# do-mpc/do-mpc

Hardware: AMD Instinct MI355X
Metric: MPC steps/sec (make_step wall-time), industrial_poly robust multi-stage (higher is better)
Workload: dtype f64

## Files before the change

__graft_entry__.py:

```python
import os
import subprocess
import sys

ROOT = os.path.dirname(os.path.abspath(__file__))
if ROOT not in sys.path:
    sys.path.insert(0, ROOT)

PREBUILT = [
    ("oscillating_masses", {}),
    ("batch_reactor", {}),
    ("batch_reactor", {"n_horizon": 50}),
    ("CSTR", {}),
    ("CSTR", {"n_robust": 0, "collocation_deg": 3}),
    ("CSTR", {"track_sign": -3000.0}),
    ("industrial_poly", {}),
    ("industrial_poly", {"n_robust": 2, "uncertainty": "paired"}),
    ("industrial_poly", {"collocation_deg": 3, "collocation_ni": 2, "n_horizon": 6}),
    ("kinematic_bicycle", {}),
    ("dynamic_bicycle", {}),
    ("kite", {"n_horizon": 20}),
    ("rotating_masses", {}),
    ("CSTR", {"custom_rterm": "default_as_expression"}),
    ("CSTR", {"custom_rterm": "custom"}),
    ("oscillating_masses", {"custom_rterm": "custom"}),
    ("oscillating_masses_dae", {}),
    ("dip", {}),
    ("CSTR", {"n_robust": 0, "nl_cons_check_colloc_points": True}),
    ("dip", {"n_horizon": 40, "nl_cons_check_colloc_points": True}),
    ("CSTR", {"nl_cons_single_slack": True}),
    ("CSTR", {"nl_cons_single_slack": True, "n_robust": 2, "n_horizon": 8, "uncertainty": {"alpha": [1.0, 1.05, 0.95], "beta": [1.0]}}),
    ("CSTR", {"nl_cons_single_slack": True, "n_robust": 0, "nl_cons_check_colloc_points": True}),
    ("CSTR", {"open_loop": True, "uncertainty": {"alpha": [1.0, 1.05, 0.95], "beta": [1.0]}}),
    ("CSTR", {"open_loop": True, "n_robust": 2, "n_horizon": 6, "uncertainty": {"alpha": [1.0, 1.05], "beta": [1.0]}, "soft_T_R": False}),
    ("shape_family:s1", {}), ("shape_family:s2", {}), ("shape_family:s3", {}), ("shape_family:s4", {}), ("shape_family:s5", {}),
    ("shape_family:s6", {}), ("shape_family:s7", {}), ("shape_family:s8", {}), ("shape_family:s9", {}),
]

PREBUILT_BATCH = [
    ("industrial_poly", {}), ("industrial_poly", {"n_robust": 2, "uncertainty": "paired"}),
    ("oscillating_masses", {}), ("CSTR", {}), ("CSTR", {"n_robust": 0, "collocation_deg": 3}), ("batch_reactor", {}), ("batch_reactor", {"n_horizon": 50}),
    ("rotating_masses", {}),
]
PREBUILT_BATCH_MHE = [("rotating_masses", "build_mhe", {}, {}), ("rotating_masses", "build_mhe_w", {"process_noise": True}, {}),
                      ("rotating_masses", "build_mhe_w", {"process_noise": True}, {"scaling": "MHE_W_SCALING"})]


PREBUILT_DEFS = [("CSTR", {}, "DOMPC_FORCE_DENSE=1"), ("batch_reactor", {}, "DOMPC_FORCE_DENSE=1"),
                 ("CSTR", {}, "DOMPC_GJ_U=1e9"), ("industrial_poly", {}, "DOMPC_GJ_U=1e9"),
                 ("batch_reactor", {}, "DOMPC_REG_GJ=0"), ("batch_reactor", {}, "DOMPC_GJ_U=1e9"),
                 ("industrial_poly", {}, "DOMPC_QUAD=0"), ("CSTR", {}, "DOMPC_QUAD=0"), ("CSTR", {"n_horizon": 5, "n_robust": 0}, "DOMPC_QUAD=0")]

PREBUILT_NODE_PACK = [("industrial_poly", {}), ("CSTR", {})] + [("shape_family:s%d" % i, {}) for i in range(1, 10)]
PREBUILT_BATCH_FAMILY = [("shape_family:s%d" % i, {}) for i in range(1, 10)]

PREBUILT_QUAD_LDS = [("DOMPC_QUAD_LDS=1", [("industrial_poly", {}), ("CSTR", {})]),
                     ("DOMPC_GJ_U=1e9", [("industrial_poly", {})]),
                     ("DOMPC_GJ_U=1e9 DOMPC_QUAD_LDS=1", [("industrial_poly", {})])]


PREBUILT_SHARD = [
    ("CSTR", {}),
    ("industrial_poly", {"n_robust": 2, "uncertainty": "paired"}),
]


PREBUILT_MHE = [("rotating_masses", "build_mhe", {}, {}), ("rotating_masses", "build_mhe_w", {"process_noise": True}, {}),
                ("rotating_masses", "build_mhe_w", {"process_noise": True}, {"scaling": "MHE_W_SCALING"}),
                ("rotating_masses", "build_mhe", {"dae": True}, {}), ("rotating_masses", "build_mhe_w", {"process_noise": True, "dae": True}, {}),
                ("oscillating_masses", "build_mhe", {"estimation": True}, {}), ("oscillating_masses", "build_mhe", {"estimation": True, "dae": True}, {}),
                ("rotating_masses", "build_mhe_w", {"process_noise": True}, {"soft_limit": (-0.1, 0.01)}),
                ("rotating_masses", "build_mhe_w", {"process_noise": True}, {"soft_limit": (-0.1, 0.01), "nl_cons_single_slack": True}),
                ("rotating_masses", "build_mhe_w", {"process_noise": True, "input_meas_noise": False}, {})]


PREBUILT_ROUTE = [("oscillating_masses", "docstring", False, False), ("oscillating_masses", "tree", False, False),
                  ("industrial_poly", "tree", False, True), ("CSTR", "tree", False, True), ("batch_reactor", "tree", False, False),
                  ("oscillating_masses_dae", "tree", False, False), ("rotating_masses", "tree", False, False),
                  ("CSTR", "docstring", False, False), ("batch_reactor", "docstring", False, False), ("industrial_poly", "docstring", False, False),
                  ("oscillating_masses", None, True, False), ("CSTR", None, True, False), ("CSTR", "tree", True, False),
                  ("industrial_poly", None, True, False), ("industrial_poly", "tree", True, False), ("batch_reactor", None, True, False),
                  ("rotating_masses", None, True, False)]


def lowered_route_cases():
    from do_mpc_amd import controller
    from do_mpc_amd.examples import CASES
    tests = os.path.join(ROOT, "tests")
    if tests not in sys.path:
        sys.path.insert(0, tests)
    import route_cases as rc
    out = []
    orig = controller.HipIpmSolver
    controller.HipIpmSolver = _NoSolver
    try:
        for name, cost, rows, batch in PREBUILT_ROUTE:
            ex = CASES[name]
            mpc = rc.stopped_before_setup(lambda n: ex.build_mpc(ex.build_model()), name)
            mpc.prepare_nlp()
            if rows:
                rc.rows_at_three_nodes(mpc, name)
            if cost:
                rc.ADDED_COST[cost](mpc)
            mpc.create_nlp()
            out.append((f"{name} + {cost or ''}{' + rows' if rows else ''} (low-level route)", {}, mpc.generated_header, mpc.model_hash, batch))
    finally:
        controller.HipIpmSolver = orig
    return out


PREBUILT_PLANTS = ["oscillating_masses", "batch_reactor", "CSTR", "industrial_poly", "oscillating_masses_dae", "dip", "rotating_masses",
                   "triple_tank", "batch_reactor_lqr_dae", "batch_reactor_lqr_dae:build_dae_model"]

PREBUILT_EKF = [("triple_tank", {}), ("oscillating_masses", {"estimation": True}), ("rotating_masses", {}), ("CSTR", {})]


def lowered_ekf(entries=None):
    from do_mpc_amd.ekf import EKF
    from do_mpc_amd.examples import CASES
    out = []
    for name, kw in (PREBUILT_EKF if entries is None else entries):
        hdr = EKF(CASES[name].build_model(**kw))._lower()
        out.append((name, kw, hdr, hdr.rsplit('EKF_MODEL_HASH "', 1)[1].split('"')[0]))
    return out


PREBUILT_EKF_DAE = ["masses", "nonlinear_discrete", "continuous", "dip", "batch_reactor", "limit", "status", "oscillating_masses_dae",
                    "masses_eliminated", "batch_reactor_eliminated"]


def lowered_ekf_dae(entries=None):
    tests = os.path.join(ROOT, "tests")
    if tests not in sys.path:
        sys.path.insert(0, tests)
    import ekf_dae_common as dc
    out = []
    for name in (PREBUILT_EKF_DAE if entries is None else entries):
        hdr = dc.make_filter(name)._lower()
        out.append((name, hdr, hdr.rsplit('EKF_MODEL_HASH "', 1)[1].split('"')[0]))
    return out


# ... 68 lines not shown

def lowered_asmpc(entries=None):
    from do_mpc_amd import lowering
    out = []
    for nx, nu in (PREBUILT_ASMPC if entries is None else entries):
        hdr = lowering.lower_asmpc(nx, nu)
        out.append((f"n_x = {nx}, n_u = {nu}", hdr, hdr.rsplit('ASMPC_MODEL_HASH "', 1)[1].split('"')[0]))
    return out


class _NoSolver:

    def __init__(self, *a, **k):
        pass


def lowered_models(which=None):
    from do_mpc_amd import controller
    from do_mpc_amd.examples import CASES
    out = []
    orig = controller.HipIpmSolver
    controller.HipIpmSolver = _NoSolver
    try:
        for name, kw in (PREBUILT if which is None else which):
            ex = CASES[name]
            mpc = ex.build_mpc(ex.build_model(), **kw)
            out.append((name, kw, mpc.generated_header, mpc.model_hash))
        if which is None:
            out += _lower_mhe(PREBUILT_MHE)
    finally:
        controller.HipIpmSolver = orig
    return out


def _lower_mhe(entries):
    from do_mpc_amd.examples import CASES
    out = []
    for name, builder, mkw, bkw in entries:
        ex = CASES[name]
        bkw = {k: (getattr(ex, v) if isinstance(v, str) else v) for k, v in bkw.items()}
        mhe = getattr(ex, builder)(ex.build_model(**mkw), **bkw)
        out.append((f"{name} ({builder})", {**mkw, **{k: "..." for k in bkw}}, mhe._mpc.generated_header, mhe._mpc.model_hash))
    return out


def lowered_mhe(entries):
    from do_mpc_amd import controller
    orig = controller.HipIpmSolver
    controller.HipIpmSolver = _NoSolver
    try:
        return _lower_mhe(entries)
    finally:
        controller.HipIpmSolver = orig


def build() -> None:
    from do_mpc_amd import build as nb
    import do_mpc_amd
    from concurrent.futures import ThreadPoolExecutor
    lib = nb.runtime_library()
    print("[build] runtime:", lib)
    jobs = [(name, kw, header, h, False, False) for name, kw, header, h in lowered_models()]
    jobs += [(name, kw, header, h, True, False) for name, kw, header, h in lowered_models(PREBUILT_SHARD)]
    jobs += [(name, kw, header, h, False, True) for name, kw, header, h in lowered_models(PREBUILT_BATCH + PREBUILT_BATCH_FAMILY)]
    jobs += [(name, kw, header, h, False, True) for name, kw, header, h in lowered_mhe(PREBUILT_BATCH_MHE)]
    route = lowered_route_cases()
    jobs += [(name, kw, header, h, False, False) for name, kw, header, h, _ in route]
    jobs += [(name, kw, header, h, False, True) for name, kw, header, h, batch in route if batch]
    with ThreadPoolExecutor(max_workers=max(1, min(len(jobs), (os.cpu_count() or 2) - 1))) as pool:
        outs = list(pool.map(lambda j: nb.model_code_object(j[2], j[3], shard=j[4], batch_only=j[5]), jobs))
    for (name, kw, _, _, shard, batch), co in zip(jobs, outs):
        print(f"[build] {name} {kw}{' (tree sharding)' if shard else ''}{' (batch only)' if batch else ''}: {co}")
    for name, kw, defs in PREBUILT_DEFS:
        saved = os.environ.get("DOMPC_DEFS")
        os.environ["DOMPC_DEFS"] = defs
        try:
            for _, _, header, h in lowered_models([(name, kw)]):
                print(f"[build] {name} {kw} [{defs}]: {nb.model_code_object(header, h)}")
        finally:
            if saved is None:
                del os.environ["DOMPC_DEFS"]
            else:
                os.environ["DOMPC_DEFS"] = saved
    for defs, classes in [("DOMPC_NODE_PACK=0", PREBUILT_NODE_PACK)] + PREBUILT_QUAD_LDS:
        saved = os.environ.get("DOMPC_DEFS")
        os.environ["DOMPC_DEFS"] = defs
        try:
            jobs = [(name, kw, header, h, batch) for name, kw, header, h in lowered_models(classes) for batch in (False, True)]
            with ThreadPoolExecutor(max_workers=max(1, min(len(jobs), (os.cpu_count() or 2) - 1))) as pool:
                outs = list(pool.map(lambda j: nb.model_code_object(j[2], j[3], batch_only=j[4]), jobs))
            for (name, kw, _, _, batch), co in zip(jobs, outs):
                print(f"[build] {name} {kw} [{defs}]{' (batch only)' if batch else ''}: {co}")
        finally:
            if saved is None:
                del os.environ["DOMPC_DEFS"]
            else:
                os.environ["DOMPC_DEFS"] = saved
    from do_mpc_amd.examples import CASES
    from do_mpc_amd.simulator import Simulator
    for name in PREBUILT_PLANTS:
        case, _, builder = name.partition(":")
        hdr = Simulator(getattr(CASES[case], builder or "build_model")())._lower()
        co = nb.plant_code_object(hdr, hdr.rsplit('PLANT_MODEL_HASH "', 1)[1].split('"')[0])
        print(f"[build] plant {name}: {co}")
    failed = []
    for entry in PREBUILT_EKF:
        try:
            for name, kw, hdr, h in lowered_ekf([entry]):
                print(f"[build] filter {name} {kw}: {nb.ekf_code_object(hdr, h)}")
        except Exception as e:
            failed.append(entry)
            print(f"[build] filter {entry[0]} {entry[1]}: FAILED\n{e}")
    for entry in PREBUILT_EKF_DAE:
        try:
            for name, hdr, h in lowered_ekf_dae([entry]):
                print(f"[build] filter of a model with algebraic states '{name}': {nb.ekf_code_object(hdr, h)}")
        except Exception as e:
            failed.append(entry)
            print(f"[build] filter of a model with algebraic states '{entry}': FAILED\n{e}")
    failed_lqr = []
    for entry in PREBUILT_LQR:
        try:
            for label, hdr, h in lowered_lqr([entry]):
                print(f"[build] LQR design {label}: {nb.lqr_code_object(hdr, h)}")
        except Exception as e:
            failed_lqr.append(entry)
            print(f"[build] LQR design {entry}: FAILED\n{e}")
    failed_ampc = []
    for entry in PREBUILT_AMPC:
        try:
            for label, hdr, h in lowered_ampc([entry]):
                print(f"[build] approximate MPC network {label}: {nb.ampc_code_object(hdr, h)}")
        except Exception as e:
            failed_ampc.append(entry)
            print(f"[build] approximate MPC network {entry}: FAILED\n{e}")
    failed_asmpc = []
    for entry in PREBUILT_ASMPC:
        try:
            for label, hdr, h in lowered_asmpc([entry]):
                print(f"[build] sensitivity-based MPC law {label}: {nb.asmpc_code_object(hdr, h)}")
        except Exception as e:
            failed_asmpc.append(entry)
            print(f"[build] sensitivity-based MPC law {entry}: FAILED\n{e}")
    mk = os.path.join(ROOT, "oracle", "Makefile")
    if os.path.exists(mk):
        subprocess.run(["make", "-C", os.path.join(ROOT, "oracle")], check=True)
    if failed:
        raise RuntimeError(f"extended Kalman filter code objects that could not be built: {failed}")
    if failed_lqr:
        raise RuntimeError(f"LQR design code objects that could not be built: {failed_lqr}")
    if failed_ampc:
        raise RuntimeError(f"approximate MPC code objects that could not be built: {failed_ampc}")
    if failed_asmpc:
        raise RuntimeError(f"sensitivity-based MPC law code objects that could not be built: {failed_asmpc}")


def smoke() -> None:
    import numpy as np
    from do_mpc_amd.examples import CASES
    from oracle import ipm
    from oracle.models import CASES as ORACLE_CASES
    from oracle.nlp import OracleNLP
    for name in ("oscillating_masses", "batch_reactor"):
        ex = CASES[name]
        mpc = ex.build_mpc(ex.build_model())
        mpc.x0 = ex.X0
        mpc.set_initial_guess()
# ... 57 lines not shown
```

do_mpc_amd/csrc/dompc_edge.h:

```cpp

template <bool SPLIT>
DOMPC_DEV inline double eval_edge_f_t(const Prob& Q, int e, const double* xv, const double* sv, double* cv, int part) {
  constexpr int REST = NI * DEG;
  const KArgs& A = *Q.A;
  const int n = A.edge_parent[e], cn = A.edge_child[e], k = A.edge_level[e];
  const double* xn = xv + A.node_x_off[n];
  const double* un = xv + A.node_u_off[n];
  const double* xc = xv + A.node_x_off[cn];
  const double* w = xv + A.edge_w_off[e];
  const double* pp = Q.P + A.p_off_p + A.edge_pidx[e] * NP;
  const double* tvp = Q.P + A.p_off_tvp + k * NTVP;
  const int row0 = A.edge_row0[e];
  const double om = A.edge_omega[e] * Q.sf;
  double f[NX];
  if (M == 0) {
    dompc_dyn_f(xn, un, nullptr, tvp, pp, f);
    double rl[NX];
    for (int a = 0; a < NX; ++a) rl[a] = f[a] - xc[a];
    for (int a = 0; a < NX; ++a) cv[row0 + a] = rl[a];
  } else {
    (void)REST;
    for (int i = 0; i < NI; ++i) {
      const double* xi0 = (i == 0) ? xn : w + slot_of(i, 0) * NX;
      const int rb = row0 + i * (DEG + 1) * NX;
// ... 143 lines not shown
constexpr bool TILE_CONDENSE = false;
#endif
constexpr int EL_MX = 0;
constexpr int GJ_LDS = (NI == 1 && DEG >= 1) ? 4 * (((DEG * NX + 3) / 4) * 4) + 256 : 0;
constexpr int EL_T1 = EL_MX + (NW * MX_LD > GJ_LDS ? NW * MX_LD : GJ_LDS);
constexpr int EL_T0 = EL_T1 + (TILE_CONDENSE ? NW : NW * NA);
constexpr int EL_RW = EL_T0 + NW;
constexpr int EL_SG = EL_RW + NW;
constexpr int EL_BB = EL_SG + NW;
constexpr int EL_QV = EL_BB + NW;
constexpr int EL_U1 = EL_QV + 2 * NA;
constexpr int EL_HUU = EL_U1 + (TILE_CONDENSE ? 0 : NU * NA + NU);
constexpr int EL_QT = EL_HUU + (TILE_CONDENSE ? 0 : NU * NU);
constexpr int EL_HP = EL_QT;
constexpr int EL_NHP = TILE_CONDENSE ? 0 : (NI * DEG > 2 ? NI * DEG : 2);
constexpr int EL_PV = EL_QT + EL_NHP * NA * NA;
constexpr int EL_RY = EL_PV + NW;
constexpr int EL_RT = EL_RY + NA;
constexpr bool R16_ENABLED = (NYT <= 16) && (NV <= 4) && (NE <= 4) && (DOMPC_SHARD == 0) && !RT_CUSTOM && !FREE_ROOT;
#ifndef DOMPC_HOST_EMU
constexpr bool RB_IN_LDS = !R16_ENABLED;
#else
constexpr bool RB_IN_LDS = true;
#endif
constexpr int RB_NEED = RB_IN_LDS ? 2 * (NYT * NYT + NYT) + 5 * NA * NA + 6 * NA + NV * NA + NV + NE * (NA + 4) : 0;
constexpr int RF_NEED = 3 * NA + NV + NX + 3 * NW1 + (NV * NA + NV) + 2 * (NX * NA + NX);
constexpr int R16_STAGE = ((ES_QV + NA + 127) / 128) * 128;
constexpr int R16_NEED = R16_ENABLED ? 2 * R16_STAGE : 0;
constexpr int el_max(int a, int b) { return a > b ? a : b; }
#ifndef DOMPC_HOST_EMU
constexpr bool MO_LDS = MO_COMPACT;
#else
constexpr bool MO_LDS = false;
#endif
constexpr int MO_IMG = MO_COMPACT ? MO_SIZE : 0;
constexpr int MOC_STAGE = MO_LDS ? ((MOC_SIZE + 127) / 128) * 128 : 0;
constexpr int EL_MOS = ((EL_RT + RT_LEN + 1) / 2) * 2;
constexpr int EL_MOC = EL_MOS + MO_IMG;
constexpr int RF_EW = ((RF_NEED + 1) / 2) * 2;
constexpr int EW_STAGE = MO_LDS ? ((EW_SIZE + 127) / 128) * 128 : 0;
constexpr int RF_MOC = RF_EW + EW_STAGE;
constexpr int RF_IMG = RF_MOC + MOC_STAGE;
constexpr int MOH_H0 = NX + NX * NA;
constexpr int DAE_NEED = DENSE_EDGE ? NW * (NW + NA + 2) + (NW + NA) * (NW + NA) + (NW + NA) * (NA + 2) + 2 * (NW + NA) + 3 * NW
                                      + NX * NW + NX * NA + NX + NE * NW + NE * NA + 2 * NW + RT_LEN : 0;
#ifndef DOMPC_QUAD
#define DOMPC_QUAD 1
#endif
#ifndef DOMPC_HOST_EMU
constexpr bool QUAD_EDGE = (DOMPC_QUAD != 0) && MO_COMPACT && (DEG >= 1) && (NA + 2 <= 16) && (NE <= 4) && !RT_CUSTOM && !FREE_ROOT &&
                           (DOMPC_SHARD == 0) && (DEG * DEG * NX <= 64) && (DOMPC_DYN_NV >= NX);
#else
constexpr bool QUAD_EDGE = false;
#endif
#ifndef DOMPC_ADJ_MU
#define DOMPC_ADJ_MU 10.0
#endif
constexpr bool QUAD_FWD = QUAD_EDGE;
DOMPC_DEV inline bool lu_store_rule(const KArgs& A, double mu, int soc) {
  if (!QUAD_FWD || (soc & 4)) return true;
  if (soc & 2) return false;
  const double thr = DOMPC_ADJ_MU * A.opt.tol;
  return mu > 0.0 && mu <= fmax(thr / A.opt.kappa_mu, pow(thr, 1.0 / A.opt.theta_mu));
}

constexpr int QL_MOSZ = QUAD_EDGE ? ((4 * MO_REC + 127) / 128) * 128 : 0;
constexpr int QL_WS = NA + 1;
constexpr int QL_WBG = ((NX * QL_WS + 1) / 2) * 2;
constexpr int QL_WB = 2 * QL_MOSZ;
constexpr int QL_VG = ((2 * NW + 7) / 8) * 8;
constexpr int QL_RW = QL_WB + 4 * QL_WBG;
constexpr int QL_QV = QL_RW + 4 * QL_VG;
constexpr int qf_pad4(int n) { return n + ((4 - n % 16) + 16) % 16; }
constexpr int QF_VG = qf_pad4(2 * NW + NA + DEG * NX);
constexpr int QF_NEED = QUAD_FWD ? QL_WB + 4 * QF_VG : 0;
constexpr int QL_NEED = QUAD_EDGE ? el_max(QL_QV + 4 * 32, QF_NEED) : 0;
constexpr int FW4_CH = ((3 * 16 + (NV * NA + NV) + 2 * (NX * NA + NX) + 1) / 2) * 2;
#ifndef DOMPC_HOST_EMU
constexpr int FW4_NEED = (NA <= 16 && NV <= 16) ? 4 * FW4_CH : 0;
#else
constexpr int FW4_NEED = 0;
#endif
constexpr int EL_SIZE = ((el_max(el_max(el_max(el_max(el_max(EL_MOC + MOC_STAGE, RB_NEED), el_max(RF_IMG + MO_IMG, R16_NEED)), DAE_NEED), QL_NEED), FW4_NEED) + 7) / 8) * 8;

DOMPC_DEV inline int moc_dense_index(int k) {
  constexpr int NVD = DOMPC_DYN_NV > 0 ? DOMPC_DYN_NV : 1;
  if (k < MOC_LT) return MO_PT + (k / NVD) * PT_STRIDE + DOMPC_DYN_VIDX[k % NVD];
  if (k < MOC_MT) return MO_LT + DOMPC_LT_VIDX[k - MOC_LT];
  if (k < MOC_NL) return MO_MT + DOMPC_MT_VIDX[k - MOC_MT];
  return MO_NL + DOMPC_NL_VIDX[k - MOC_NL];
}
constexpr int MOC_PL = (MOC_N + GS_C - 1) / GS_C > 0 ? (MOC_N + GS_C - 1) / GS_C : 1;
struct MocMap { int idx[MOC_PL]; };
DOMPC_DEV inline MocMap moc_map(int lane, int GS) {
  MocMap m;
#pragma unroll
  for (int q = 0; q < MOC_PL; ++q) {
    const int k = lane + q * GS;
    m.idx[q] = moc_dense_index(k < MOC_N ? k : 0);
  }
  return m;
}
DOMPC_DEV inline void mo_image_init(ldsd* img, int lane, int GS) {
  for (int i = lane; i < MO_SIZE; i += GS) img[i] = 0.0;
#ifndef DOMPC_HOST_EMU
  __builtin_amdgcn_fence(__ATOMIC_ACQ_REL, "wavefront");
  __builtin_amdgcn_wave_barrier();
#endif
  for (int i = lane; i < NCOLL * DOMPC_DYN_NC; i += GS)
    img[MO_PT + (i / (DOMPC_DYN_NC > 0 ? DOMPC_DYN_NC : 1)) * PT_STRIDE + DOMPC_DYN_CIDX[i % (DOMPC_DYN_NC > 0 ? DOMPC_DYN_NC : 1)]] =
        DOMPC_DYN_CVAL[i % (DOMPC_DYN_NC > 0 ? DOMPC_DYN_NC : 1)];
  for (int i = lane; i < DOMPC_LT_NC; i += GS) img[MO_LT + DOMPC_LT_CIDX[i]] = DOMPC_LT_CVAL[i];
  for (int i = lane; i < DOMPC_MT_NC; i += GS) img[MO_MT + DOMPC_MT_CIDX[i]] = DOMPC_MT_CVAL[i];
  for (int i = lane; i < DOMPC_NL_NC; i += GS) img[MO_NL + DOMPC_NL_CIDX[i]] = DOMPC_NL_CVAL[i];
#ifndef DOMPC_HOST_EMU
  __builtin_amdgcn_fence(__ATOMIC_ACQ_REL, "wavefront");
  __builtin_amdgcn_wave_barrier();
#endif
}
template <class SRC>
DOMPC_DEV inline void mo_expand(ldsd* img, SRC src, const MocMap& m, int lane, int GS) {
#pragma unroll
  for (int q = 0; q < MOC_PL; ++q) {
    const int k = lane + q * GS;
    if (k < MOC_N) img[m.idx[q]] = src[k];
  }
#ifndef DOMPC_HOST_EMU
  __builtin_amdgcn_fence(__ATOMIC_ACQ_REL, "wavefront");
  __builtin_amdgcn_wave_barrier();
#endif
}

DOMPC_DEV inline int point_of_slot(int sl) {
  if (sl < DEG) return sl;
  const int s2 = sl - DEG, i = 1 + s2 / (DEG + 1), r = s2 % (DEG + 1);
  return (r == 0 || i >= NI) ? -1 : i * DEG + r - 1;
}

DOMPC_DEV inline void dyn_c_noalias(const double* __restrict__ xs, const double* __restrict__ us, const double* __restrict__ tvp,
                                    const double* __restrict__ pp, const double* __restrict__ lam, double* __restrict__ o) {
  dompc_dyn_c(xs, us, nullptr, tvp, pp, lam, o);
}
DOMPC_DEV inline void lterm_c_noalias(const double* __restrict__ xs, const double* __restrict__ us, const double* __restrict__ tvp,
                                      const double* __restrict__ pp, double* __restrict__ o) {
  dompc_lterm_c(xs, us, nullptr, tvp, pp, o);
}
DOMPC_DEV inline void mterm_c_noalias(const double* __restrict__ xs, const double* __restrict__ tvp, const double* __restrict__ pp, double* __restrict__ o) {
  dompc_mterm_c(xs, tvp, pp, o);
}
DOMPC_PHASE void eval_models(const Thr& T, const Prob& Q) {
  const KArgs& A = *Q.A;
  constexpr int NPT = NPT_E;
  const int E = A.n_edges;
  const int e_last0 = E - (A.level_node_start[A.N + 1] - A.level_node_start[A.N]);
  const int n_dyn = E * NPT, n_lt = E, n_mt = E - e_last0, n_nl = (NE > 0) ? E : 0;
  for (int it = T.tid; it < n_dyn + n_lt + n_mt + n_nl; it += T.nt) {
    int kind, e, j = 0;
    if (it < n_dyn) { kind = 0; e = it / NPT; j = it % NPT; }
    else if (it < n_dyn + n_lt) { kind = 1; e = it - n_dyn; }
    else if (it < n_dyn + n_lt + n_mt) { kind = 2; e = e_last0 + (it - n_dyn - n_lt); }
    else { kind = 3; e = it - n_dyn - n_lt - n_mt; }
    if (!mk_e(A, e)) continue;
    if constexpr (DENSE_EDGE) { dae_eval_item(Q, kind, e, j); continue; }
    const int n = A.edge_parent[e], cn = A.edge_child[e], k = A.edge_level[e];
    const double* xn = Q.x + A.node_x_off[n];
    const double* un = Q.x + A.node_u_off[n];
// ... 76 lines not shown
```

do_mpc_amd/csrc/dompc_quad.h:

```cpp
#if !defined(DOMPC_HOST_EMU) && DOMPC_DEG >= 1 && DOMPC_M >= 1 && DOMPC_NI == 1 && DOMPC_NX + DOMPC_NU + 2 <= 16 && DOMPC_DEG * DOMPC_DEG * DOMPC_NX <= 64

using dompc_lanes::rbc;
using dompc_lanes::pin;
using dompc_lanes::fmac_rbc;
using dompc_lanes::dpp_ready;
using dompc_lanes::sfor;

struct MoRef { int kind, off; };
constexpr MoRef moref_in(int d, const int* vidx, int nv, const int* cidx, int nc, int base) {
  for (int k = 0; k < nv; ++k) if (vidx[k] == d) return MoRef{2, base + k};
  for (int k = 0; k < nc; ++k) if (cidx[k] == d) return MoRef{1, k};
  return MoRef{0, 0};
}
constexpr MoRef moref_dyn(int p, int d) { return moref_in(d, DOMPC_DYN_VIDX, DOMPC_DYN_NV, DOMPC_DYN_CIDX, DOMPC_DYN_NC, p * DOMPC_DYN_NV); }
constexpr MoRef moref_lt(int d) { return moref_in(d, DOMPC_LT_VIDX, DOMPC_LT_NV, DOMPC_LT_CIDX, DOMPC_LT_NC, MOC_LT); }
constexpr MoRef moref_nl(int d) { return moref_in(d, DOMPC_NL_VIDX, DOMPC_NL_NV, DOMPC_NL_CIDX, DOMPC_NL_NC, MOC_NL); }
constexpr MoRef moref_mt(int d) { return moref_in(d, DOMPC_MT_VIDX, DOMPC_MT_NV, DOMPC_MT_CIDX, DOMPC_MT_NC, MOC_MT); }
template <int KIND, int OFF>
__device__ inline double mo_dyn_val(const ldsd* rec) { if constexpr (KIND == 2) return rec[OFF]; else if constexpr (KIND == 1) return DOMPC_DYN_CVAL[OFF]; else return 0.0; }
template <int KIND, int OFF>
__device__ inline double mo_lt_val(const ldsd* rec) { if constexpr (KIND == 2) return rec[OFF]; else if constexpr (KIND == 1) return DOMPC_LT_CVAL[OFF]; else return 0.0; }
template <int KIND, int OFF>
__device__ inline double mo_nl_val(const ldsd* rec) { if constexpr (KIND == 2) return rec[OFF]; else if constexpr (KIND == 1) return DOMPC_NL_CVAL[OFF]; else return 0.0; }
template <int KIND, int OFF>
// ... 607 lines not shown
    constexpr int s = S_;
    sfor<R>([&](auto R_) {
      constexpr int r = R_, jj = r / NX, a = r % NX;
      double v = 0.0;
      if constexpr (s == jj)
        sfor<NX>([&](auto B_) {
          constexpr int bb = B_;
          constexpr MoRef rf = moref_dyn(jj, NX + a * NA + bb);
          if constexpr (rf.kind != 0) { const double t_ = mo_dyn_val<rf.kind, rf.off>(rec); v = (j == bb) ? t_ : v; }
        });
      if constexpr (s == 0) {
        sfor<NU>([&](auto K_) {
          constexpr int ku = K_;
          constexpr MoRef rf = moref_dyn(jj, NX + a * NA + NX + ku);
          if constexpr (rf.kind != 0) { const double t_ = mo_dyn_val<rf.kind, rf.off>(rec); v = (j == NX + ku) ? t_ : v; }
        });
        const double rb_ = rbc<a>(res[jj]);
        v = (j == NA) ? rb_ : v;
      }
      v = (j == a) ? v - DOMPC_C[(s + 1) * (DEG + 1) + jj + 1] : v;
      bc[s][r] = v;
    });
  });
}
__device__ inline int qd_fw_eliminate(int j, double (&bc)[DEG][DEG * NX]) {
  constexpr int R = DEG * NX;
  constexpr double GJ_U = DOMPC_GJ_U;
  int bad = 0;
  double sig[DEG];
#pragma unroll
  for (int s = 0; s < DEG; ++s) sig[s] = 1.0;
  sfor<R>([&](auto K_) {
    constexpr int k = K_, sk = k / NX, bk = k % NX;
    constexpr int rt1 = (4 * (k / 4 + 1) < R) ? 4 * (k / 4 + 1) : R;
    QD_SB();
    const bool own = (j == bk);
    double m = 0.0;
#pragma unroll
    for (int r = k + 1; r < rt1; ++r) m = fmax(m, fabs(bc[sk][r]));
    const double akk = fabs(bc[sk][k]);
    bad |= (int)(own & !(akk >= GJ_U * m && akk > 1e-300));
    const double pl = fast_rcp((akk > 1e-300) ? bc[sk][k] : 1.0);
    const double pinv = rbc<bk>(pl);
    sig[sk] = own ? -pl : sig[sk];
    double pm[DEG];
#pragma unroll
    for (int s = 0; s < DEG; ++s) {
      const double prow = bc[s][k] * pinv;
      pm[s] = (s == sk && own) ? 0.0 : -prow;
      bc[s][k] = (s == sk && own) ? -1.0 : prow;
      pin(pm[s]);
    }
    asm volatile("s_nop 1");
    sfor<R>([&](auto R_) {
      constexpr int r = R_;
      if constexpr (r != k) {
        sfor<DEG>([&](auto S_) { constexpr int s = S_; if constexpr (s != sk) fmac_rbc<bk>(bc[s][r], bc[sk][r], pm[s]); });
        fmac_rbc<bk>(bc[sk][r], bc[sk][r], pm[sk]);
      }
    });
#pragma unroll
    for (int s = 0; s < DEG; ++s)
#pragma unroll
      for (int r = 0; r < R; ++r) pin(bc[s][r]);
  });
  QD_SB();
#pragma unroll
  for (int s = 0; s < DEG; ++s)
#pragma unroll
    for (int r = 0; r < R; ++r) bc[s][r] *= sig[s];
  QD_SB();
  return bad;
}

struct QfPack { int woff, row0, level, n, cn, uoffp, epsoff; };
__device__ inline QfPack qf_pack(const KArgs& A, int e) {
  const auto* ep = A.edge_pack + e * EP_N;
  QfPack k;
  k.woff = ep[EP_WOFF]; k.row0 = ep[EP_ROW0]; k.level = ep[EP_LEVEL]; k.n = ep[EP_PARENT]; k.cn = ep[EP_CHILD];
  k.uoffp = ep[EP_UOFF_PARENT]; k.epsoff = ep[EP_EPSOFF_PARENT];
  return k;
}

__device__ __attribute__((noinline)) void phase_forward_quads(const void* kp, int b_, int slot, int soc, double sf, double delta_, int cl_) {
  const KArgs A = kernel_args(kp);
  Thr T = make_thr(A);
  T.kp = kp;
  Prob Q = make_prob(A, ufl(slot), A.p + (int64_t)ufl(b_) * A.n_opt_p);
  Q.sf = ufl(sf);
  Q.soc = ufl(soc);
  prob_bounds(Q);
  const double delta = ufl(delta_);
  const int cl = ufl(cl_);
  (void)delta;
  constexpr int R = DEG * NX;
  const int ng = T.nt / 64, gid = group_index(T.tid, 64);
  ldsd* Ld = T.edge_lds + (int64_t)(T.ltid / 64) * EL_SIZE;
  const int nq = (A.n_edges + 3) / 4;
  int bank = 0;
  int qd = gid;
  if (qd >= nq) return;
  {
    const int lane0 = (int)(threadIdx.x & 63u);
    stage_quad(Q, 4 * qd, lane0, Ld, 0);
  }
#if DOMPC_QUAD_PROFILE
  long long pc0 = prof_clock();
#define QF_PH(i) if (T.prof && T.tid == 0) { const long long pc1 = prof_clock(); T.prof[i] += pc1 - pc0; pc0 = pc1; }
#else
#define QF_PH(i)
#endif
  while (qd < nq) {
    int lane = (int)(threadIdx.x & 63u);
    asm volatile("" : "+v"(lane));
    const int g = lane >> 4, j = lane & 15;
    const int e0 = 4 * qd;
    const bool act = e0 + g < A.n_edges;
    const int e = act ? e0 + g : A.n_edges - 1;
    const bool isx = j < NX, st_x = act && isx;
    const int b = isx ? j : 0;
    const QfPack pk = qf_pack(A, e);
    const bool chain = pk.level >= cl;
    const double dxn = Q.nd[(int64_t)pk.n * ND_SIZE + ND_DXT + b];
    double du[NU > 0 ? NU : 1];
#pragma unroll
    for (int u = 0; u < NU; ++u) du[u] = Q.dx[pk.uoffp + u];
    double cres[DEG], rwv[M], sgv[M];
#pragma unroll
    for (int jj = 0; jj < DEG; ++jj) cres[jj] = Q.c[pk.row0 + jj * NX + b];
    const double ccont = Q.c[pk.row0 + R + b];
    const double* ew = Q.ew + (int64_t)e * EW_SIZE;
#pragma unroll
    for (int s = 0; s < M; ++s) { rwv[s] = ew[EW_RW + s * NX + b]; sgv[s] = ew[EW_SIGW + s * NX + b]; }
    double dnu = Q.dlam[pk.row0 + NW + b];
    if (__ballot(!chain) != 0ull) {
      const double* Nc = Q.nd + (int64_t)pk.cn * ND_SIZE;
      double t = Nc[ND_PV + b];
#pragma unroll
      for (int bb = 0; bb < NA; ++bb) t = fma(Nc[ND_P + b * NA + bb], Nc[ND_DXT + bb], t);
      dnu = chain ? dnu : t;
    }
    asm volatile("s_waitcnt vmcnt(0)" ::: "memory");
    __builtin_amdgcn_fence(__ATOMIC_ACQ_REL, "wavefront");
    __builtin_amdgcn_wave_barrier();
    QF_PH(15)
    const ldsd* rec = Ld + bank * QL_MOSZ + (e - e0) * MO_REC;
    ldsd* Lv = Ld + QL_WB + g * QF_VG;
    constexpr int V_DW = 0, V_DY = NW, V_RHS = NW + NA, V_RR = 2 * NW + NA;
    if (isx) Lv[V_DY + j] = dxn;
    sfor<NU>([&](auto U_) { constexpr int u = U_; if (j == NX + u) Lv[V_DY + NX + u] = du[u]; });
    double gv[DEG];
    sfor<DEG>([&](auto J_) {
      constexpr int jj = J_;
      double t = cres[jj] - DOMPC_C[0 * (DEG + 1) + jj + 1] * dxn;
      sfor<NX>([&](auto A_) {
        constexpr int a = A_;
        sfor<NU>([&](auto U_) {
          constexpr int u = U_;
          constexpr MoRef rf = moref_dyn(jj, NX + a * NA + NX + u);
          if constexpr (rf.kind != 0) { const double t_ = mo_dyn_val<rf.kind, rf.off>(rec) * du[u]; t += (j == a) ? t_ : 0.0; }
        });
      });
      gv[jj] = t;
      pin(gv[jj]);
    });
    QD_SB();
    double bc[DEG][R];
    qd_fw_columns(rec, j, gv, bc);
    QF_PH(28)
    QD_SB();
    const int bad = qd_fw_eliminate(j, bc);
    const bool fb = __ballot(bad) != 0ull;
    QF_PH(29)
    const int qn = qd + ng;
    if (qn < nq) stage_quad(Q, 4 * qn, lane, Ld, bank ^ 1);
    double dwv[M];
    if (!fb) {
#pragma unroll
      for (int s = 0; s < DEG; ++s) dwv[s] = 0.0;
      sfor<R>([&](auto R_) {
        constexpr int r = R_, s = r / NX, a = r % NX;
        const double t_ = rbc<NA>(bc[0][r]);
        dwv[s] = (j == a) ? -t_ : dwv[s];
      });
    } else {
      __builtin_amdgcn_fence(__ATOMIC_ACQ_REL, "wavefront");
      __builtin_amdgcn_wave_barrier();
      if (isx) {
#pragma unroll
        for (int s = 0; s < DEG; ++s) Lv[V_RR + s * NX + j] = gv[s];
      }
      __builtin_amdgcn_fence(__ATOMIC_ACQ_REL, "wavefront");
      __builtin_amdgcn_wave_barrier();
#pragma unroll
      for (int s = 0; s < DEG; ++s) {
        double t = 0.0;
        for (int k2 = 0; k2 < R; ++k2) t -= ew[EW_LU + (s * NX + b) * LU_N + k2] * Lv[V_RR + k2];
        dwv[s] = t;
      }
      __builtin_amdgcn_fence(__ATOMIC_ACQ_REL, "wavefront");
      __builtin_amdgcn_wave_barrier();
    }
    {
      double t = DOMPC_D[0] * dxn - ccont;
#pragma unroll
      for (int s = 1; s <= DEG; ++s) t = fma(DOMPC_D[s], dwv[s - 1], t);
      dwv[M - 1] = t;
    }
    if (isx) {
#pragma unroll
      for (int s = 0; s < M; ++s) Lv[V_DW + s * NX + j] = dwv[s];
    }
    __builtin_amdgcn_fence(__ATOMIC_ACQ_REL, "wavefront");
    __builtin_amdgcn_wave_barrier();
    QF_PH(30)
    QD_SB();
    double rhs[M];
    sfor<M>([&](auto S_) {
      constexpr int s = S_;
      double t = fma(sgv[s], dwv[s], rwv[s]);
      if constexpr (s == M - 1) t += dnu;
      if constexpr (s < DEG) {
        sfor<NA>([&](auto I_) {
          constexpr int i = I_;
          sfor<NA - i>([&](auto D_) {
            constexpr int k = i + D_;
            constexpr MoRef rf = moref_dyn(s, MOH_H0 + symi(i, k, NA));
            if constexpr (rf.kind != 0 && i < NX) {
              const double h = mo_dyn_val<rf.kind, rf.off>(rec);
              if constexpr (k < NX) {
                const double pk_ = h * (double)Lv[V_DW + s * NX + k];
                t += (j == i) ? pk_ : 0.0;
                if constexpr (i != k) { const double pi_ = h * (double)Lv[V_DW + s * NX + i]; t += (j == k) ? pi_ : 0.0; }
              } else {
                const double pu_ = h * du[k - NX];
                t += (j == i) ? pu_ : 0.0;
              }
            }
          });
        });
      }
      rhs[s] = -t;
      pin(rhs[s]);
    });
    QF_PH(31)
    QD_SB();
    if (isx) {
#pragma unroll
      for (int s = 0; s < DEG; ++s) Lv[V_RR + s * NX + j] = fma(DOMPC_D[s + 1], rhs[M - 1], rhs[s]);
    }
    __builtin_amdgcn_fence(__ATOMIC_ACQ_REL, "wavefront");
    __builtin_amdgcn_wave_barrier();
    double dl[M];
    if (!fb) {
#pragma unroll
      for (int s = 0; s < DEG; ++s) {
        double t = 0.0;
#pragma unroll
        for (int k2 = 0; k2 < R; ++k2) t = fma(bc[s][k2], (double)Lv[V_RR + k2], t);
        dl[s] = t;
      }
    } else {
#pragma unroll
      for (int s = 0; s < DEG; ++s) {
        double t = 0.0;
        for (int k2 = 0; k2 < R; ++k2) t += ew[EW_LU + k2 * LU_N + s * NX + b] * Lv[V_RR + k2];
        dl[s] = t;
      }
    }
    dl[M - 1] = rhs[M - 1];
    if (st_x) {
#pragma unroll
      for (int s = 0; s < M; ++s) {
        Q.dx[pk.woff + s * NX + j] = dwv[s];
        Q.dlam[pk.row0 + s * NX + j] = dl[s];
      }
      if (!chain) Q.dlam[pk.row0 + NW + j] = dnu;
    }
    if constexpr (NE > 0) {
      if (act && j < NE) {
        const double* S_ = Q.es + (int64_t)e * ES_SIZE;
        double t = S_[ES_RDN + j];
        for (int bb = 0; bb < NA; ++bb) t += ew[EW_JD + j * NA + bb] * Lv[V_DY + bb];
        if (!EPS_GLOBAL && nl_slack(j) >= 0) t -= Q.sgn[e * NE1 + j] * Q.dx[pk.epsoff + nl_slack(j)];
        Q.ds[e * NE1 + j] = t;
        Q.dlam[pk.row0 + NW + NX + j] = (S_[ES_SIGS + j] + delta) * t + S_[ES_RSN + j];
      }
    }
    __builtin_amdgcn_fence(__ATOMIC_ACQ_REL, "wavefront");
    __builtin_amdgcn_wave_barrier();
    QF_PH(20)
    bank ^= 1;
    qd = qn;
  }
#undef QF_PH
}
#elif !defined(DOMPC_HOST_EMU)
__device__ inline void phase_forward_quads(const void*, int, int, int, double, double, int) {}
#endif
```

Before: 11510.

## Prefetch forward-quad operands into LDS one quad ahead via global_load_lds

In the forward-quad phase, each edge's index record is fetched one quad ahead and broadcast across lanes with DPP and readlane. The per-edge operands (Sigma_w and r_w, residuals c, dx, dnu, du) are staged into LDS with async global_load_lds during the previous iteration, so their global-load latency overlaps compute instead of sitting in the critical path before the wait. Eligibility is gated by constexpr size checks, and the old path can be restored with DOMPC_FWD_STAGE=0. The risks are extra LDS footprint, an added lgkmcnt wait, and subtle correctness reliance on buffer reuse timing.

```diff
diff --git a/__graft_entry__.py b/__graft_entry__.py
--- a/__graft_entry__.py
+++ b/__graft_entry__.py
@@ -57,6 +57,8 @@
                      ("DOMPC_GJ_U=1e9", [("industrial_poly", {})]),
                      ("DOMPC_GJ_U=1e9 DOMPC_QUAD_LDS=1", [("industrial_poly", {})])]
 
+PREBUILT_FWD_STAGE = [("DOMPC_FWD_STAGE=0", [("industrial_poly", {}), ("CSTR", {})]),
+                      ("DOMPC_GJ_U=1e9 DOMPC_FWD_STAGE=0", [("industrial_poly", {})])]
 
 PREBUILT_SHARD = [
     ("CSTR", {}),
@@ -291,7 +293,7 @@
                 del os.environ["DOMPC_DEFS"]
             else:
                 os.environ["DOMPC_DEFS"] = saved
-    for defs, classes in [("DOMPC_NODE_PACK=0", PREBUILT_NODE_PACK)] + PREBUILT_QUAD_LDS:
+    for defs, classes in [("DOMPC_NODE_PACK=0", PREBUILT_NODE_PACK)] + PREBUILT_QUAD_LDS + PREBUILT_FWD_STAGE:
         saved = os.environ.get("DOMPC_DEFS")
         os.environ["DOMPC_DEFS"] = defs
         try:
diff --git a/do_mpc_amd/csrc/dompc_edge.h b/do_mpc_amd/csrc/dompc_edge.h
--- a/do_mpc_amd/csrc/dompc_edge.h
+++ b/do_mpc_amd/csrc/dompc_edge.h
@@ -249,6 +249,12 @@
 constexpr int FW4_NEED = 0;
 #endif
 constexpr int EL_SIZE = ((el_max(el_max(el_max(el_max(el_max(EL_MOC + MOC_STAGE, RB_NEED), el_max(RF_IMG + MO_IMG, R16_NEED)), DAE_NEED), QL_NEED), FW4_NEED) + 7) / 8) * 8;
+#ifndef DOMPC_FWD_STAGE
+#define DOMPC_FWD_STAGE 1
+#endif
+constexpr int QF_SG = QF_NEED;
+constexpr int QF_SG_EW = 0, QF_SG_C = QF_SG_EW + 4 * 64, QF_SG_V = QF_SG_C + 4 * 32, QF_SG_SIZE = QF_SG_V + 4 * 32;
+constexpr bool QF_STAGE = QUAD_FWD && (DOMPC_FWD_STAGE != 0) && NW <= 32 && 2 * NX + NU <= 32 && QF_SG % 2 == 0 && QF_SG + QF_SG_SIZE <= EL_SIZE;
 
 DOMPC_DEV inline int moc_dense_index(int k) {
   constexpr int NVD = DOMPC_DYN_NV > 0 ? DOMPC_DYN_NV : 1;
diff --git a/do_mpc_amd/csrc/dompc_quad.h b/do_mpc_amd/csrc/dompc_quad.h
--- a/do_mpc_amd/csrc/dompc_quad.h
+++ b/do_mpc_amd/csrc/dompc_quad.h
@@ -713,6 +713,47 @@
   return k;
 }
 
+constexpr bool QF_STAGED = QF_STAGE && EW_SIGW % 2 == 0;
+static_assert(EP_N == 16, "one index record per row of 16 lanes");
+__device__ inline int qf_index_request(const KArgs& A, int e0, int lane) {
+  const int e = min(e0 + (lane >> 4), A.n_edges - 1);
+  return A.edge_pack[(int64_t)e * EP_N + (lane & 15)];
+}
+template <int F>
+__device__ inline int qf_row_field(int ipk) { return __builtin_amdgcn_update_dpp(0, ipk, 0x150 + F, 0xf, 0xf, true); }
+__device__ inline void qf_glds4(const double* src, int word, ldsd* dst) {
+  __builtin_amdgcn_global_load_lds((const __attribute__((address_space(1))) void*)((const unsigned*)src + word),
+                                   (__attribute__((address_space(3))) void*)dst, 4, 0, 0);
+}
+__device__ inline void stage_quad_operands(const Prob& Q, int e0, int ipk, int lane, ldsd* Ld) {
+  const KArgs& A = *Q.A;
+  ldsd* dst = Ld + QF_SG;
+  static_assert(EW_RW == EW_SIGW + NW, "Sigma_w | r_w is one run of 2 NW doubles");
+  static_assert(!QF_STAGED || (EW_SIGW % 2 == 0 && EW_SIZE % 8 == 0 && QF_SG % 2 == 0), "16-byte pieces of Sigma_w | r_w, in memory and in LDS");
+#pragma unroll
+  for (int p = 0; p < 2; ++p) {
+    const int e = min(e0 + 2 * p + (lane >> 5), A.n_edges - 1);
+    const double* src = Q.ew + (int64_t)e * EW_SIZE + EW_SIGW + 2 * min(lane & 31, NW - 1);
+    __builtin_amdgcn_global_load_lds((const __attribute__((address_space(1))) void*)src,
+                                     (__attribute__((address_space(3))) void*)(dst + QF_SG_EW + 128 * p), 16, 0, 0);
+  }
+  const int k = min(lane >> 1, 2 * NX + NU - 1), h = lane & 1;
+  sfor<4>([&](auto G_) {
+    constexpr int gg = G_;
+    const int row0 = __builtin_amdgcn_readlane(ipk, 16 * gg + EP_ROW0), n = __builtin_amdgcn_readlane(ipk, 16 * gg + EP_PARENT);
+    qf_glds4(Q.c + row0, min(lane, 2 * NW - 1), dst + QF_SG_C + 32 * gg);
+    const double* xs = Q.nd + (int64_t)n * ND_SIZE + ND_DXT + k;
+    const double* ns = Q.dlam + row0 + NW + (k - NX);
+    const double* vs = k < NX ? xs : ns;
+    if constexpr (NU > 0) {
+      const int uoffp = __builtin_amdgcn_readlane(ipk, 16 * gg + EP_UOFF_PARENT);
+      const double* us = Q.dx + uoffp + (k - 2 * NX);
+      vs = k < 2 * NX ? vs : us;
+    }
+    qf_glds4(vs, h, dst + QF_SG_V + 32 * gg);
+  });
+}
+
 __device__ __attribute__((noinline)) void phase_forward_quads(const void* kp, int b_, int slot, int soc, double sf, double delta_, int cl_) {
   const KArgs A = kernel_args(kp);
   Thr T = make_thr(A);
@@ -735,6 +776,12 @@
     const int lane0 = (int)(threadIdx.x & 63u);
     stage_quad(Q, 4 * qd, lane0, Ld, 0);
   }
+  int ipk = 0, ipkn = 0;
+  if constexpr (QF_STAGED) {
+    const int lane0 = (int)(threadIdx.x & 63u);
+    ipk = qf_index_request(A, 4 * qd, lane0);
+    stage_quad_operands(Q, 4 * qd, ipk, lane0, Ld);
+  }
 #if DOMPC_QUAD_PROFILE
   long long pc0 = prof_clock();
 #define QF_PH(i) if (T.prof && T.tid == 0) { const long long pc1 = prof_clock(); T.prof[i] += pc1 - pc0; pc0 = pc1; }
@@ -750,20 +797,31 @@
     const int e = act ? e0 + g : A.n_edges - 1;
     const bool isx = j < NX, st_x = act && isx;
     const int b = isx ? j : 0;
-    const QfPack pk = qf_pack(A, e);
+    QfPack pk;
+    if constexpr (QF_STAGED) {
+      pk.woff = qf_row_field<EP_WOFF>(ipk); pk.row0 = qf_row_field<EP_ROW0>(ipk); pk.level = qf_row_field<EP_LEVEL>(ipk);
+      pk.n = 0; pk.cn = qf_row_field<EP_CHILD>(ipk); pk.uoffp = 0; pk.epsoff = qf_row_field<EP_EPSOFF_PARENT>(ipk);
+    } else {
+      pk = qf_pack(A, e);
+    }
     const bool chain = pk.level >= cl;
-    const double dxn = Q.nd[(int64_t)pk.n * ND_SIZE + ND_DXT + b];
+    double dxn, ccont, dnu;
     double du[NU > 0 ? NU : 1];
-#pragma unroll
-    for (int u = 0; u < NU; ++u) du[u] = Q.dx[pk.uoffp + u];
     double cres[DEG], rwv[M], sgv[M];
-#pragma unroll
-    for (int jj = 0; jj < DEG; ++jj) cres[jj] = Q.c[pk.row0 + jj * NX + b];
-    const double ccont = Q.c[pk.row0 + R + b];
     const double* ew = Q.ew + (int64_t)e * EW_SIZE;
-#pragma unroll
-    for (int s = 0; s < M; ++s) { rwv[s] = ew[EW_RW + s * NX + b]; sgv[s] = ew[EW_SIGW + s * NX + b]; }
-    double dnu = Q.dlam[pk.row0 + NW + b];
+    if constexpr (!QF_STAGED) {
+      dxn = Q.nd[(int64_t)pk.n * ND_SIZE + ND_DXT + b];
+#pragma unroll
+      for (int u = 0; u < NU; ++u) du[u] = Q.dx[pk.uoffp + u];
+#pragma unroll
+      for (int jj = 0; jj < DEG; ++jj) cres[jj] = Q.c[pk.row0 + jj * NX + b];
+      ccont = Q.c[pk.row0 + R + b];
+#pragma unroll
+      for (int s = 0; s < M; ++s) { rwv[s] = ew[EW_RW + s * NX + b]; sgv[s] = ew[EW_SIGW + s * NX + b]; }
+      dnu = Q.dlam[pk.row0 + NW + b];
+    } else {
+      dnu = 0.0;
+    }
     if (__ballot(!chain) != 0ull) {
       const double* Nc = Q.nd + (int64_t)pk.cn * ND_SIZE;
       double t = Nc[ND_PV + b];
@@ -771,10 +829,25 @@
       for (int bb = 0; bb < NA; ++bb) t = fma(Nc[ND_P + b * NA + bb], Nc[ND_DXT + bb], t);
       dnu = chain ? dnu : t;
     }
+    if constexpr (!QF_STAGED) { QF_PH(17) }
     asm volatile("s_waitcnt vmcnt(0)" ::: "memory");
     __builtin_amdgcn_fence(__ATOMIC_ACQ_REL, "wavefront");
     __builtin_amdgcn_wave_barrier();
     QF_PH(15)
+    if constexpr (QF_STAGED) {
+      if (qd + ng < nq) ipkn = qf_index_request(A, 4 * (qd + ng), lane);
+      const ldsd* So = Ld + QF_SG;
+      dxn = So[QF_SG_V + 32 * g + b];
+      const double dnus = So[QF_SG_V + 32 * g + NX + b];
+      dnu = chain ? dnus : dnu;
+#pragma unroll
+      for (int u = 0; u < NU; ++u) du[u] = So[QF_SG_V + 32 * g + 2 * NX + u];
+#pragma unroll
+      for (int jj = 0; jj < DEG; ++jj) cres[jj] = So[QF_SG_C + 32 * g + jj * NX + b];
+      ccont = So[QF_SG_C + 32 * g + R + b];
+#pragma unroll
+      for (int s = 0; s < M; ++s) { rwv[s] = So[QF_SG_EW + 64 * g + NW + s * NX + b]; sgv[s] = So[QF_SG_EW + 64 * g + s * NX + b]; }
+    }
     const ldsd* rec = Ld + bank * QL_MOSZ + (e - e0) * MO_REC;
     ldsd* Lv = Ld + QL_WB + g * QF_VG;
     constexpr int V_DW = 0, V_DY = NW, V_RHS = NW + NA, V_RR = 2 * NW + NA;
@@ -805,6 +878,13 @@
     QF_PH(29)
     const int qn = qd + ng;
     if (qn < nq) stage_quad(Q, 4 * qn, lane, Ld, bank ^ 1);
+    if constexpr (QF_STAGED) {
+      if (qn < nq) {
+        asm volatile("s_waitcnt lgkmcnt(0)" ::: "memory");
+        stage_quad_operands(Q, 4 * qn, ipkn, lane, Ld);
+      }
+      QF_PH(17)
+    }
     double dwv[M];
     if (!fb) {
 #pragma unroll
@@ -923,6 +1003,7 @@
     QF_PH(20)
     bank ^= 1;
     qd = qn;
+    ipk = ipkn;
   }
 #undef QF_PH
 }
```

Measured after the change: 11770 (median of 6 runs). 1.02x the previous value.
